# ZhiHuangHn/vtkCloudPoint

Measured on AMD Instinct MI355X. Metric: Mpoints/s DBSCAN+label @10M pts, higher is better.
Workload: dtype f64; 1 GPU; C4: 10000000-pt cloud (half uniform background, 200 Gaussian blobs), one monolithic DBImproved.dbscan, metric L1_2D, eps 0.1, minPts 10; mode=single, points_total=10000000, points_per_gpu=10000000, clusters=27380, resident_in_hbm=True

## Files before the change

### vtkcloudpoint_amd/csrc/dbscan.hip

```cpp
#include <string.h>

#include <cmath>
#include <cstdlib>
#include <cstring>
#include <limits>
#include <vector>

#include "bounds.hpp"
#include "dbscan_engine.hpp"
#include "grid_common.hpp"

using namespace vcpg;

namespace {

#ifndef VCP_UNR2
#define VCP_UNR2 4
#endif
#ifndef VCP_UNR3
#define VCP_UNR3 2
#endif
#ifndef VCP_UNRW
#define VCP_UNRW 4
#endif
// ... 814 lines not shown
template <bool FILTER>
__global__ __launch_bounds__(TPB) void k_flatten(uint32_t* __restrict__ parent, const uint32_t* __restrict__ sord,
                                                uint32_t* __restrict__ minord, WorkList wlE) {
  const uint32_t p = wl_fetch(wlE);
  uint32_t r = NONE, v = NONE;
  if (p != NONE) {
    r = (uint32_t)p;
    uint32_t x = parent[r];
    while (x != r) {
      r = x;
      x = parent[r];
    }
    parent[p] = r;
    v = sord[p];
  }
  unsigned long long todo = __ballot(r != NONE);
  const int lane = threadIdx.x & 63;
  while (todo) {
    int leader = __ffsll((long long)todo) - 1;
    uint32_t lr = __shfl(r, leader, 64);
    bool mine = (r == lr);
    uint32_t m = mine ? v : NONE;
#pragma unroll
    for (int d = 32; d > 0; d >>= 1) m = min(m, (uint32_t)__shfl_xor((int)m, d, 64));
    if (lane == leader &&
        (!FILTER || m < __hip_atomic_load(&minord[lr], __ATOMIC_RELAXED, __HIP_MEMORY_SCOPE_AGENT)))
      atomicMin(&minord[lr], m);
    todo &= ~__ballot(mine);
  }
}

__device__ __forceinline__ uint32_t seed_rank(const uint32_t* __restrict__ bits, const uint32_t* __restrict__ pref,
                                              uint32_t m) {
  const uint32_t w = m >> 5;
  return pref[w] + (uint32_t)__popc(bits[w] & ((1u << (m & 31u)) - 1u));
}
__global__ __launch_bounds__(TPB) void k_seed_popc(const uint32_t* __restrict__ bits, uint32_t nw, uint32_t* __restrict__ cnt) {
  uint32_t w = blockIdx.x * TPB + threadIdx.x;
  if (w < nw) cnt[w] = (uint32_t)__popc(bits[w]);
}

__global__ __launch_bounds__(TPB) void k_seedflag(const uint32_t* __restrict__ parent, const uint32_t* __restrict__ minord,
                                                 uint32_t* __restrict__ seedflag, WorkList wlE) {
  const uint32_t p = wl_fetch(wlE);
  if (p == NONE) return;
  if (parent[p] == p) {
    const uint32_t m = minord[p];
    atomicOr(&seedflag[m >> 5], 1u << (m & 31u));
  }
}

__global__ __launch_bounds__(TPB) void k_rootk(const uint32_t* __restrict__ parent, const uint32_t* __restrict__ minord,
                                              const uint32_t* __restrict__ seedbits, const uint32_t* __restrict__ seedpref,
                                              uint32_t* __restrict__ rootk, uint32_t* __restrict__ clseed, WorkList wlE) {
  const uint32_t p = wl_fetch(wlE);
  if (p == NONE) return;
  if (parent[p] == p) {
    uint32_t k = seed_rank(seedbits, seedpref, minord[p]);
    rootk[p] = k;
    clseed[k] = minord[p];
  }
}

__device__ __forceinline__ void twice_add(unsigned twice, unsigned long long* __restrict__ counters) {
  __shared__ unsigned tw[TPB / 64];
  const unsigned long long m2 = __ballot(twice);
  if ((threadIdx.x & 63) == 0) tw[threadIdx.x >> 6] = (unsigned)__popcll(m2);
  __syncthreads();
  if (threadIdx.x == 0) {
    unsigned t = 0;
    for (int k = 0; k < TPB / 64; k++) t += tw[k];
    if (t) atomicAdd(&counters[36 + (blockIdx.x & 31)], (unsigned long long)t);
  }
}

template <int GD, int METRIC, bool GROUPED>
__global__ __launch_bounds__(TPB) void k_border(ExactSrc xs, GridP g, double thr,
                                               CellTab ct,
                                               const int32_t* __restrict__ sgroup, const uint8_t* __restrict__ flags,
                                               const uint32_t* __restrict__ parent, const uint32_t* __restrict__ sord,
                                               const uint32_t* __restrict__ rootk, const uint32_t* __restrict__ clseed,
                                               uint32_t* __restrict__ labk, unsigned long long* __restrict__ counters,
                                               uint32_t* __restrict__ group_twice, WorkList wlB, uint32_t own_lo,
                                               uint32_t own_span, const float* __restrict__ sorted32, Screen sc) {
  const uint32_t p = wl_fetch(wlB);
  unsigned twice = 0;
  if (p != NONE) {
    const uint8_t fl = flags[p];
    uint32_t out = 0;
    {
      float qf[3];
      int cc[3];
      load_pt32<GD>(sorted32, p, qf);
      cell_of32<GD>(qf, g, cc);
      constexpr int UNR = VCP_UNRW;
      const int32_t myg = GROUPED ? sgroup[p] : 0;
      uint32_t mx = 0, mnk = NONE;
      for_rows<GD>(cc, g, ct, [&](uint32_t s, uint32_t e) {
        for (uint32_t j0 = s; j0 < e; j0 += UNR) {
          uint32_t rk[UNR];
#pragma unroll
          for (int u = 0; u < UNR; u++) rk[u] = rootk[min(j0 + u, e - 1)];
#pragma unroll
          for (int u = 0; u < UNR; u++) {
            const uint32_t j = j0 + u, x = rk[u];
            if (j >= e || x == NONE || (x >= mnk && x < mx)) continue;
            if (GROUPED && sgroup[j] != myg) continue;
            float rr[3];
            load_pt32<GD>(sorted32, j, rr);
            if (within_scr<GD, METRIC>(qf, rr, sc, xs, p, j, thr)) {
              mx = max(mx, x + 1u);
              mnk = min(mnk, x);
            }
          }
        }
        return true;
      });
      out = mx;
      if (mx != 0 && !(fl & F_CLASSED) && sord[p] - own_lo < own_span && sord[p] < clseed[mnk]) {
        twice = 1;
        if (GROUPED) atomicAdd(&group_twice[myg], 1u);
      }
    }
    labk[p] = (out << 2) | ((fl & F_CORE) ? 1u : 0u) | ((fl & F_CLASSED) ? 2u : 0u);
  }
  if (!GROUPED) twice_add(twice, counters);
}

template <bool GROUPED>
__global__ __launch_bounds__(TPB) void k_border_list(const int32_t* __restrict__ sgroup, const uint8_t* __restrict__ flags,
                                                    const uint32_t* __restrict__ sord, const uint32_t* __restrict__ rootk,
                                                    const uint32_t* __restrict__ clseed, uint32_t* __restrict__ labk,
                                                    unsigned long long* __restrict__ counters,
                                                    uint32_t* __restrict__ group_twice, NbrOut no, WorkList wlB) {
  const uint32_t p = wl_fetch(wlB);
  unsigned twice = 0;
  if (p != NONE) {
    const uint8_t fl = flags[p];
    const int nrec = fl >> 4;
    uint32_t mx = 0, mnk = NONE;
    const uint32_t* li = nbr_list(no, p);
    for (int k = 0; k < nrec; k++) {
      const uint32_t x = rootk[li[k]];
      if (x == NONE) continue;
      mx = max(mx, x + 1u);
      mnk = min(mnk, x);
    }
    if (mx != 0 && sord[p] < clseed[mnk]) twice = 1;
    labk[p] = (mx << 2) | ((fl & F_CORE) ? 1u : 0u) | ((fl & F_CLASSED) ? 2u : 0u);
  }
  if (GROUPED) {
    const int32_t g = twice ? sgroup[p] : -1;
    unsigned long long todo = __ballot(twice != 0);
    const int lane = threadIdx.x & 63;
    while (todo) {
      const int leader = __ffsll((long long)todo) - 1;
      const int32_t gl = __shfl(g, leader, 64);
      const unsigned long long same = __ballot(twice && g == gl);
      if (lane == leader) atomicAdd(&group_twice[gl], (uint32_t)__popcll(same));
      todo &= ~same;
    }
  } else {
    twice_add(twice, counters);
  }
}

__global__ __launch_bounds__(TPB) void k_labk_rest(const uint8_t* __restrict__ flags, const uint32_t* __restrict__ parent,
                                                  uint32_t* rootk, uint32_t* __restrict__ labk,
                                                  CellTab ct) {
  const uint32_t nin = *ct.nin;
  int64_t p = (int64_t)blockIdx.x * TPB + threadIdx.x;
  if (p >= nin) return;
  const uint8_t fl = flags[p];
  uint32_t k = NONE;
  if (fl & F_EXPAND) {
    const uint32_t r = parent[p];
    k = rootk[r];
    if (r != (uint32_t)p) rootk[p] = k;
  } else {
    rootk[p] = NONE;
  }
  if (fl & F_BCAND) return;
  const uint32_t out = (fl & F_EXPAND) ? k + 1u : 0u;
  labk[p] = (out << 2) | ((fl & F_CORE) ? 1u : 0u) | ((fl & F_CLASSED) ? 2u : 0u);
}

template <bool GROUPED>
__global__ __launch_bounds__(TPB) void k_output(int64_t n, const uint32_t* __restrict__ pos,
                                               const uint32_t* __restrict__ labk,
                                               const uint8_t* __restrict__ in_classed, const int32_t* __restrict__ group,
                                               const uint32_t* __restrict__ groupstart,
                                               const uint32_t* __restrict__ seedbits,
                                               const uint32_t* __restrict__ seedpref, int32_t cf_in,
                                               int32_t* __restrict__ labels, uint8_t* __restrict__ is_core,
                                               uint8_t* __restrict__ is_classed,
                                               unsigned long long* __restrict__ counters) {
  int64_t i = (int64_t)blockIdx.x * TPB + threadIdx.x;
  unsigned unclassed = 0;
  (void)counters;
  if (i < n) {
    const uint32_t p = pos[i];
    if (p == NONE) {
      if (GROUPED) return;
      if (!in_classed) labels[i] = 0;
      if (is_core) is_core[i] = 0;
      if (is_classed) is_classed[i] = in_classed ? in_classed[i] : 0;
    } else {
      const uint32_t w = labk[p];
      const uint32_t k1 = w >> 2;
      const bool core = w & 1u, classed = w & 2u;
      int32_t lab = 0;
      if (k1) {
        uint32_t base = GROUPED ? seed_rank(seedbits, seedpref, groupstart[group[i]]) : 0u;
        lab = cf_in + (int32_t)(k1 - base);
      }
      if (lab != 0 || !in_classed) labels[i] = lab;
      if (is_core) is_core[i] = (core && !classed) ? 1 : 0;
      if (is_classed) is_classed[i] = (classed || lab != 0) ? 1 : 0;
      if (!classed) unclassed = 1;
    }
  }
  if (in_classed) {
    __shared__ unsigned wcnt[TPB / 64];
    unsigned long long m1 = __ballot(unclassed);
    if ((threadIdx.x & 63) == 0) wcnt[threadIdx.x >> 6] = (unsigned)__popcll(m1);
    __syncthreads();
    if (threadIdx.x == 0) {
// ... 431 lines not shown
    static const int cap_env = getenv("VCP_CORE_CAP") ? atoi(getenv("VCP_CORE_CAP")) : -1;
    no.core_cap = (GD == 2 && (uint64_t)n < (uint64_t)g.ncells) ? std::min(no.NB, CORE_LIST) : no.NB;
    if (cap_env >= 0) no.core_cap = std::min(no.NB, cap_env);
  }
  const size_t lds_nb = (size_t)no.NB * TPB * 4;
  static const bool core_global = getenv("VCP_CORE_GLOBAL") != nullptr;
  if constexpr (GD == 2) {
    if (!GROUPED || !core_global)
      VCP_LAUNCH(ctx, (k_core_lds<GD, METRIC, GROUPED>), dim3(nb), dim3(TPB), 0, st, xs, g, thr, min_pts, ct, sgroup, flags,
                      parent, minord, blkE, blkB, no, sorted32, sc, flags_set);
    else
      VCP_LAUNCH(ctx, (k_core<GD, METRIC, GROUPED>), dim3(nb), dim3(TPB), 2 * lds_nb, st, xs, g, thr, min_pts, ct,
                      sgroup, flags, parent, minord, blkE, blkB, no, sorted32, sc, flags_set);
  } else
    VCP_LAUNCH(ctx, (k_core<GD, METRIC, GROUPED>), dim3(nb), dim3(TPB), 2 * lds_nb, st, xs, g, thr, min_pts, ct,
                    sgroup, flags, parent, minord, blkE, blkB, no, sorted32, sc, flags_set);
  VCP_TRY(vcp_exclusive_scan_u32(ctx, blkE, blkE, 2 * ((int64_t)nb + 2), nullptr));
  VCP_LAUNCH(ctx, k_wl_fill, dim3(nb), dim3(TPB), 0, st, flags, ct, blkE, blkB, wlE.list, wlB.list,
                  seedflag, nw, counters, GROUPED ? ext->d_group_twice : nullptr, (uint32_t)(GROUPED ? G : 0));

  vcp_phase(ctx, "union");
  const bool pre = GD == 2 || no.NB > 0;
  if (no.NB > 0) {
    VCP_LAUNCH(ctx, k_union_init_list, dim3(nbl), dim3(TPB), 0, st, flags, parent, no, wlE);
    static const int join_all = getenv("VCP_JOIN_ALL") ? atoi(getenv("VCP_JOIN_ALL")) : -1;
    const bool all = join_all >= 0 ? join_all != 0 : (uint64_t)n >= (uint64_t)g.ncells;
    if (all) VCP_LAUNCH(ctx, k_flatten0<2>, dim3(nbl), dim3(TPB), 0, st, parent, wlE, flags, no);
    else VCP_LAUNCH(ctx, k_flatten0<1>, dim3(nbl), dim3(TPB), 0, st, parent, wlE, flags, no);
    VCP_LAUNCH(ctx, k_flatten0<0>, dim3(nbl), dim3(TPB), 0, st, parent, wlE, flags, no);
  } else if (GD == 2) {
    VCP_LAUNCH(ctx, (k_union_init<GD, METRIC, GROUPED>), dim3(nbl), dim3(TPB), 0, st, xs, g, thr, ct, sgroup,
                    flags, parent, wlE, sorted32, sc);
    VCP_LAUNCH(ctx, k_flatten0<0>, dim3(nbl), dim3(TPB), 0, st, parent, wlE, flags, no);
  }
  const bool dense = pre && (uint64_t)n > (uint64_t)DENSE_PER_CELL * g.ncells;
  if (dense) {
    VCP_TRY(vcp_ensure(ctx, ctx->b_aux0, ((size_t)nb * (TPB / 64) + 2) * 4));
    uint32_t* chunkroot = ctx->b_aux0.as<uint32_t>();
    VCP_LAUNCH(ctx, k_chunkroot, dim3(nb), dim3(TPB), 0, st, parent, ct, chunkroot);
    VCP_LAUNCH(ctx, (k_union<GD, METRIC, GROUPED, true, true>), dim3(nbl), dim3(TPB), 0, st, xs, g, thr, ct, sgroup,
                    parent, wlE, sorted32, sc, chunkroot);
  } else if (pre)
    VCP_LAUNCH(ctx, (k_union<GD, METRIC, GROUPED, true>), dim3(nbl), dim3(TPB), 0, st, xs, g, thr, ct, sgroup,
                    parent, wlE, sorted32, sc);
  else
    VCP_LAUNCH(ctx, (k_union<GD, METRIC, GROUPED, false>), dim3(nbl), dim3(TPB), 0, st, xs, g, thr, ct, sgroup,
                    parent, wlE, sorted32, sc);
  vcp_phase(ctx, "flatten_number");
  if ((uint64_t)n >= (uint64_t)g.ncells)
    VCP_LAUNCH(ctx, k_flatten<true>, dim3(nbl), dim3(TPB), 0, st, parent, sord, minord, wlE);
  else
    VCP_LAUNCH(ctx, k_flatten<false>, dim3(nbl), dim3(TPB), 0, st, parent, sord, minord, wlE);
  if (!GROUPED && ext && ext->slab) {
    vcp_phase(ctx, "slab_components");
    VCP_LAUNCH(ctx, k_slab_count, dim3(nb), dim3(TPB), 0, st, parent, flags, ct, blkE);
    VCP_TRY(vcp_exclusive_scan_u32(ctx, blkE, blkE, (int64_t)nb + 1, nullptr));
    VCP_LAUNCH(ctx, k_slab_fill, dim3(nb), dim3(TPB), 0, st, parent, flags, minord, ct, blkE, clseed);
    VCP_LAUNCH(ctx, k_slab_out, dim3(nb), dim3(TPB), 0, st, n, pos, flags, parent, minord, ext->d_slab_rep, d_is_core);
    uint32_t* hn = reinterpret_cast<uint32_t*>(ctx->pinned) + 64;
    VCP_HIP(ctx, hipMemcpyAsync(hn, blkE + nb, 4, hipMemcpyDeviceToHost, st));
    VCP_TRY(vcp_phase_finish(ctx));
    VCP_HIP(ctx, hipStreamSynchronize(st));
    if (!ctx->slab) ctx->slab = new SlabState();
    SlabState& ss = *ctx->slab;
    ss.valid = true;
    ss.gd = GD;
    ss.metric = METRIC;
    ss.n = n;
    ss.n_comp = hn[0];
    ss.g = g;
    ss.thr = thr;
    ss.sc = sc;
    ss.xs = xs;
    ss.nb = nb;
    if (cf_out) *cf_out = (int32_t)hn[0];
    return VCP_OK;
  }
  VCP_LAUNCH(ctx, k_seedflag, dim3(nbl), dim3(TPB), 0, st, parent, minord, seedflag, wlE);
  VCP_LAUNCH(ctx, k_seed_popc, dim3(vcp_blocks(nw, TPB)), dim3(TPB), 0, st, seedflag, nw, seedpref);
  VCP_TRY(vcp_exclusive_scan_u32(ctx, seedpref, seedpref, nw, d_total));
  VCP_LAUNCH(ctx, k_rootk, dim3(nbl), dim3(TPB), 0, st, parent, minord, seedflag, seedpref, rootk, clseed, wlE);

  vcp_phase(ctx, "border");
  VCP_LAUNCH(ctx, k_labk_rest, dim3(nb), dim3(TPB), 0, st, flags, parent, rootk, labk, ct);
  if (no.NB > 0)
    VCP_LAUNCH(ctx, k_border_list<GROUPED>, dim3(nbl), dim3(TPB), 0, st, sgroup, flags, sord, rootk, clseed, labk, counters,
                    GROUPED ? ext->d_group_twice : nullptr, no, wlB);
  else
    VCP_LAUNCH(ctx, (k_border<GD, METRIC, GROUPED>), dim3(nbl), dim3(TPB), 0, st, xs, g, thr, ct, sgroup, flags,
                    parent, sord, rootk, clseed, labk, counters, GROUPED ? ext->d_group_twice : nullptr, wlB, 0u, NONE,
                    sorted32, sc);
  if (part_out) {
    GridOutputArgs oa;
    oa.n = n;
    oa.sord = sord;
    oa.labk = labk;
    oa.have_in_classed = d_in_classed != nullptr;
    oa.cf_in = cf_in;
    oa.labels = d_labels;
    oa.is_core = d_is_core;
    oa.is_classed = d_is_classed;
    oa.counters = counters;
    VCP_TRY(vcp_grid_output_partition(ctx, oa));
  } else {
    vcp_phase(ctx, "output");
    VCP_LAUNCH(ctx, (k_output<GROUPED>), dim3(nb), dim3(TPB), 0, st, n, pos, labk, d_in_classed, d_group,
                    GROUPED ? ext->d_groupstart : nullptr, seedflag, seedpref, cf_in, d_labels, d_is_core, d_is_classed,
                    counters);
  }
  if (!GROUPED && min_pts <= 0 && !all_finite)
    VCP_LAUNCH(ctx, k_lonely_seeds<GD>, dim3(nb), dim3(TPB), 0, st, d_coords, n, stride, d_in_classed, d_is_classed,
                    counters);
  if (GROUPED) {
    VCP_LAUNCH(ctx, k_group_stats, dim3(vcp_blocks(G, TPB)), dim3(TPB), 0, st, G, glo, ghi, ext->d_groupstart,
                    seedflag, seedpref, ext->d_group_twice, ext->d_group_nclus, counters + 3, ext->skip_upto);
    if (ext->d_group_evals)
      VCP_HIP(ctx, hipMemcpyAsync(ext->d_group_evals, counters + 3, 8, hipMemcpyDeviceToDevice, st));
  }
  unsigned long long* hc = reinterpret_cast<unsigned long long*>(ctx->pinned) + 8;
  VCP_HIP(ctx, hipMemcpyAsync(hc, counters, 68 * sizeof(unsigned long long), hipMemcpyDeviceToHost, st));
  VCP_TRY(vcp_phase_finish(ctx));
  VCP_HIP(ctx, hipStreamSynchronize(st));
  const uint32_t K = *reinterpret_cast<uint32_t*>(hc + 2);
  unsigned long long unclassed = (unsigned long long)n;
  if (d_in_classed) {
    unclassed = 0;
    for (int k = 0; k < 32; k++) unclassed += hc[4 + k];
  }
  if (cf_out) *cf_out = cf_in + (int32_t)K;
  unsigned long long twice_total = 0;
  for (int k = 0; k < 32; k++) twice_total += hc[36 + k];
  if (dist_evals) *dist_evals = GROUPED ? (int64_t)hc[3] : (int64_t)(unclassed + twice_total + K - hc[0]) * n;
  return VCP_OK;
}

template <int GD, int METRIC>
int run_slab_finish(vcp_ctx* ctx, const SlabState& ss, const uint32_t* d_map_rep, const uint32_t* d_map_k,
                    const int32_t* d_tab_gid, uint32_t own_lo, uint32_t own_span, int32_t* d_labels,
                    uint8_t* d_is_classed, int64_t* twice) {
  hipStream_t st = ctx->stream;
  const int64_t n = ss.n;
  const unsigned nb = ss.nb;
  const GridP g = ss.g;
  const size_t ctw = vcp_ct_words(g.ncells);
  const CellTab ct{ctx->b_ctw.as<uint4>(), ctx->b_ctd.as<uint32_t>(),
                   reinterpret_cast<uint32_t*>(ctx->b_ctw.as<char>() + ctw * 16) + 1};
  uint32_t* pos = ctx->b_pos.as<uint32_t>();
  uint32_t* sord = ctx->b_sidx.as<uint32_t>();
  uint8_t* flags = ctx->b_flags.as<uint8_t>();
  uint32_t* parent = ctx->b_parent.as<uint32_t>();
  uint32_t* minord = ctx->b_minord.as<uint32_t>();
  uint32_t* rootk = ctx->b_rootcl.as<uint32_t>();
  uint32_t* clseed = ctx->b_clseed.as<uint32_t>();
  uint32_t* labk = ctx->b_labk.as<uint32_t>();
  WorkList wlB;
  uint32_t* blkE = ctx->b_wl.as<uint32_t>();
  uint32_t* blkB = blkE + (nb + 2);
  wlB.list = blkB + (nb + 2) + n;
  wlB.scan = blkB;
  wlB.nblk = nb;
  wlB.perblk = list_perblk(n);
  const unsigned nbl = 8u * LCHUNK * wlB.perblk;
  const int rb = (int)vcp_blocks(n, TPB, 1024);
  unsigned long long* counters = reinterpret_cast<unsigned long long*>(ctx->b_misc.as<double>() + (size_t)rb * 8 + 8);
  vcp_phase(ctx, "slab_roots");
  VCP_HIP(ctx, hipMemsetAsync(counters, 0, 68 * sizeof(unsigned long long), st));
  VCP_LAUNCH(ctx, k_slab_rootk, dim3(nb), dim3(TPB), 0, st, parent, flags, minord, ct, d_map_rep, d_map_k,
                  (uint32_t)ss.n_comp, rootk, counters);
  vcp_phase(ctx, "border");
  VCP_LAUNCH(ctx, k_labk_rest, dim3(nb), dim3(TPB), 0, st, flags, parent, rootk, labk, ct);
  VCP_LAUNCH(ctx, (k_border<GD, METRIC, false>), dim3(nbl), dim3(TPB), 0, st, ss.xs, g, ss.thr,
                  ct, nullptr, flags, parent, sord, rootk, clseed, labk, counters, nullptr, wlB, own_lo, own_span,
                  ctx->b_sorted32.as<float>(), ss.sc);
  vcp_phase(ctx, "output");
  VCP_LAUNCH(ctx, k_slab_output, dim3(nb), dim3(TPB), 0, st, n, pos, labk, d_tab_gid, d_labels, d_is_classed);
  unsigned long long* hc = reinterpret_cast<unsigned long long*>(ctx->pinned) + 8;
  VCP_HIP(ctx, hipMemcpyAsync(hc, counters, 68 * sizeof(unsigned long long), hipMemcpyDeviceToHost, st));
  VCP_TRY(vcp_phase_finish(ctx));
  VCP_HIP(ctx, hipStreamSynchronize(st));
  if (hc[0] != 0)
    return vcp_fail(ctx, VCP_ERR_ARG, "%llu local components are missing from the map", hc[0]);
  if (twice) {
    *twice = 0;
    for (int k = 0; k < 32; k++) *twice += (int64_t)hc[36 + k];
  }
  return VCP_OK;
}

int run_degenerate(vcp_ctx* ctx, int64_t n, int min_pts, int32_t cf_in, const uint8_t* d_in_classed,
                   int32_t* d_labels, uint8_t* d_is_core, uint8_t* d_is_classed, int32_t* cf_out,
                   int64_t* dist_evals) {
  hipStream_t st = ctx->stream;
  const unsigned nb = vcp_blocks(n, TPB);
  vcp_phase(ctx, "degenerate");
  VCP_TRY(vcp_ensure(ctx, ctx->b_seedflag, (size_t)(n + 2) * 4));
  VCP_TRY(vcp_ensure(ctx, ctx->b_misc, 64));
  uint32_t* f = ctx->b_seedflag.as<uint32_t>();
  uint32_t* d_total = ctx->b_misc.as<uint32_t>();
  VCP_LAUNCH(ctx, k_unclassed_flag, dim3(nb), dim3(TPB), 0, st, d_in_classed, f, n);
  VCP_TRY(vcp_exclusive_scan_u32(ctx, f, f, n, d_total));
  const int all_core = 0 >= min_pts;
  VCP_LAUNCH(ctx, k_degenerate, dim3(nb), dim3(TPB), 0, st, d_in_classed, f, n, cf_in, all_core,
                  d_in_classed == nullptr, d_labels, d_is_core, d_is_classed);
  uint32_t* hu = reinterpret_cast<uint32_t*>(ctx->pinned);
  VCP_HIP(ctx, hipMemcpyAsync(hu, d_total, 4, hipMemcpyDeviceToHost, st));
  VCP_TRY(vcp_phase_finish(ctx));
  VCP_HIP(ctx, hipStreamSynchronize(st));
  if (cf_out) *cf_out = cf_in + (all_core ? (int32_t)hu[0] : 0);
  if (dist_evals) *dist_evals = (int64_t)hu[0] * n;
  return VCP_OK;
}

}

int vcp_dbscan_engine(vcp_ctx* ctx, const double* d_coords, int64_t n, int stride, int metric, double eps,
                      int min_pts, int32_t cf_in, const uint8_t* d_in_classed, int32_t* d_labels,
                      uint8_t* d_is_core, uint8_t* d_is_classed, int32_t* cf_out, int64_t* dist_evals,
                      const DbscanExt* ext) {
  if (!ctx) return VCP_ERR_ARG;
  if (n < 0) return vcp_fail(ctx, VCP_ERR_ARG, "n < 0");
  if (stride != 2 && stride != 3) return vcp_fail(ctx, VCP_ERR_ARG, "dim must be 2 or 3");
  if (metric < 0 || metric > 3) return vcp_fail(ctx, VCP_ERR_ARG, "unknown metric %d", metric);
  if (metric == VCP_SIGNED_SUM_2D) {
    if (ext) return vcp_fail(ctx, VCP_ERR_ARG, "DB has no grouped / staged form");
    if (n >= 0x7FFFFFF0LL) return vcp_fail(ctx, VCP_ERR_TOO_LARGE, "n beyond 32-bit indexing");
    if (n > 0 && (!d_coords || !d_labels)) return vcp_fail(ctx, VCP_ERR_ARG, "null buffer");
    VCP_TRY(vcp_bind(ctx));
    vcp_phase_reset(ctx);
    if (ctx->slab) ctx->slab->valid = false;
    if (n == 0) {
      if (cf_out) *cf_out = cf_in;
      if (dist_evals) *dist_evals = 0;
      ctx->last_timing.clear();
      return VCP_OK;
    }
    return vcp_db_engine(ctx, d_coords, n, stride, eps, min_pts, cf_in, nullptr, d_in_classed, d_labels, d_is_core,
                         d_is_classed, cf_out, dist_evals);
  }
  if (metric == VCP_L2_3D && stride != 3) return vcp_fail(ctx, VCP_ERR_ARG, "VCP_L2_3D needs dim 3");
  if (n >= 0x3FFFFFF0LL) return vcp_fail(ctx, VCP_ERR_TOO_LARGE, "n beyond 30-bit indexing");
  if (n > 0 && (!d_coords || !d_labels)) return vcp_fail(ctx, VCP_ERR_ARG, "null buffer");
  const bool grouped = ext && ext->d_group;
  if (grouped && (metric != VCP_L1_2D || !ext->d_groupstart || !ext->d_group_twice || d_in_classed))
    return vcp_fail(ctx, VCP_ERR_ARG, "grouped DBSCAN needs groupstart, group_twice and the L1 metric");
  VCP_TRY(vcp_bind(ctx));
  vcp_phase_reset(ctx);
  if (ctx->slab) ctx->slab->valid = false;
  if (n == 0) {
    if (cf_out) *cf_out = cf_in;
    if (dist_evals) *dist_evals = 0;
    ctx->last_timing.clear();
    return VCP_OK;
  }
  if (!(eps >= 0.0)) {
    if (grouped) return vcp_fail(ctx, VCP_ERR_ARG, "grouped DBSCAN needs eps >= 0");
    return run_degenerate(ctx, n, min_pts, cf_in, d_in_classed, d_labels, d_is_core, d_is_classed, cf_out, dist_evals);
// ... 154 lines not shown
```

### vtkcloudpoint_amd/csrc/grid_common.hpp

```cpp
#pragma once
#include "vcp_ctx.hpp"

namespace vcpg {

constexpr int TPB = 256;
constexpr uint8_t F_CORE = 1, F_CLASSED = 2, F_EXPAND = 4, F_BCAND = 8;
constexpr uint32_t NONE = 0xFFFFFFFFu;

struct GridP {
  double mn[3];
  double inv_h;
  double scale;
  int D[3];
  uint32_t ncells;
};

template <int GD>
__device__ __forceinline__ uint32_t cell_id(const GridP& g, int cx, int cy, int cz) {
  uint32_t id = (uint32_t)cy * (uint32_t)g.D[0] + (uint32_t)cx;
  if (GD == 3) id += (uint32_t)cz * (uint32_t)g.D[0] * (uint32_t)g.D[1];
  return id;
}

__device__ __forceinline__ float rel32(double x, double mn, double scale) { return (float)((x - mn) * scale); }
// ... 76 lines not shown
  return t.dense[(size_t)w.w * 32u + i];
}
__device__ __forceinline__ uint32_t ct_from_word(const CellTab& t, const uint4 w, uint32_t cell) {
  const uint32_t i = cell & 31u, below = (1u << i) - 1u;
  if ((w.x & w.y & below) == 0u) return w.z + (uint32_t)__popc(w.x & below) + 2u * (uint32_t)__popc(w.y & below);
  return t.dense[(size_t)w.w * 32u + i];
}
__device__ __forceinline__ void ct_range(const CellTab& t, uint32_t c0, uint32_t c1, uint32_t& s, uint32_t& e) {
  const uint4 w0 = t.words[c0 >> 5];
  s = ct_from_word(t, w0, c0);
  e = (c1 >> 5) == (c0 >> 5) ? ct_from_word(t, w0, c1) : ct_start(t, c1);
}

struct Screen {
  float lo, hi;
};

template <int GD>
__device__ __forceinline__ void load_pt32(const float* __restrict__ c, int64_t i, float* q) {
  if (GD == 2) {
    const float2 v = *reinterpret_cast<const float2*>(c + 2 * i);
    q[0] = v.x;
    q[1] = v.y;
  } else {
    const float4 v = *reinterpret_cast<const float4*>(c + 4 * i);
    q[0] = v.x;
    q[1] = v.y;
    q[2] = v.z;
  }
}
template <int GD>
__device__ __forceinline__ void store_pt32(float* __restrict__ c, int64_t i, const double* q, const GridP& g) {
  if (GD == 2) {
    *reinterpret_cast<float2*>(c + 2 * i) = make_float2(rel32(q[0], g.mn[0], g.scale), rel32(q[1], g.mn[1], g.scale));
  } else {
    *reinterpret_cast<float4*>(c + 4 * i) =
        make_float4(rel32(q[0], g.mn[0], g.scale), rel32(q[1], g.mn[1], g.scale), rel32(q[2], g.mn[2], g.scale), 0.0f);
  }
}

struct ExactSrc {
  const double* base;
  const uint32_t* idx;
  int stride;
};
template <int GD>
__device__ __forceinline__ void load_exact(const ExactSrc& xs, uint32_t p, double* q) {
  const int64_t i = xs.idx ? (int64_t)xs.idx[p] : (int64_t)p;
  load_in<GD>(xs.base, i, xs.stride, q);
}

}

struct GridBuildArgs {
  const double* d_coords = nullptr;
  int64_t n = 0;
  int stride = 2, gd = 2;
  vcpg::GridP g;
  const int32_t* d_group = nullptr;
  int glo = 0, ghi = 0;
  const uint32_t* d_ord = nullptr;
  const uint8_t* d_in_classed = nullptr;
  uint4* ctwords = nullptr;
  uint32_t* ctdense = nullptr;
  uint32_t* ctcount = nullptr;
  float* sorted32 = nullptr;
  uint32_t* sord = nullptr;
  uint32_t* sidx = nullptr;
  int32_t* sgroup = nullptr;
  uint8_t* flags = nullptr;
  uint32_t* pos = nullptr;
};
__host__ __device__ static inline size_t vcp_ct_words(uint32_t ncells) { return ((size_t)ncells + 32) / 32; }
static inline size_t vcp_ct_dense_cap(int64_t n, uint32_t ncells) {
  const size_t w = vcp_ct_words(ncells), byn = (size_t)n / 3 + 1;
  return w < byn ? w : byn;
}
int vcp_grid_build_partition(vcp_ctx* ctx, const GridBuildArgs& a);

struct GridOutputArgs {
  int64_t n = 0;
  const uint32_t* sord = nullptr;
  const uint32_t* labk = nullptr;
  bool have_in_classed = false;
  int32_t cf_in = 0;
  int32_t* labels = nullptr;
  uint8_t* is_core = nullptr;
  uint8_t* is_classed = nullptr;
  unsigned long long* counters = nullptr;
};
int vcp_grid_output_partition(vcp_ctx* ctx, const GridOutputArgs& a);
```

### vtkcloudpoint_amd/csrc/gridbuild.hip

```cpp
#include <algorithm>
#include <mutex>
#include <unordered_map>

#include "grid_common.hpp"

using namespace vcpg;

namespace {

constexpr int PT = 1024;
constexpr int PCH_MIN = 8192;
constexpr int FT = 1024;
constexpr uint32_t MAXB = 8192;
constexpr uint32_t wcap(int) { return 4096u; }
constexpr uint32_t QUEUE_FROM = 32;

typedef float4 Rec;

template <int GD>
__device__ __forceinline__ Rec rec_make(const float* qf, uint32_t idx, uint32_t cell) {
  return GD == 2 ? make_float4(qf[0], qf[1], __uint_as_float(idx), __uint_as_float(cell))
                 : make_float4(qf[0], qf[1], qf[2], __uint_as_float(idx));
}
template <int GD>
// ... 494 lines not shown
      uint32_t i;
      const uint32_t p = cnt[padded(rec_cell<GD>(r, g, i) - c0)] + rk[j] - s - w0;
      if (p < WCAP) stage_put<GD>(s32, sidx, p, r, i);
    }
    __syncthreads();
    fine_flush<GD, GROUPED>(s + w0, min(WCAP, m - w0), s32, sidx, ord, in_classed, group, sorted32, sord, sidx_out, sgroup,
                            flags, pos);
    __syncthreads();
  }
}

template <int GD, bool GROUPED>
__global__ __launch_bounds__(FT) void k_part_fine_windows(const Rec* __restrict__ rec, const uint32_t* __restrict__ rk,
                                                         const uint32_t* __restrict__ bstart, uint32_t bstride,
                                                         const uint32_t* __restrict__ total, uint32_t B, GridP g,
                                                         const uint32_t* __restrict__ ord, const uint8_t* __restrict__ in_classed,
                                                         const int32_t* __restrict__ group, CellTab ct,
                                                         float* __restrict__ sorted32,
                                                         uint32_t* __restrict__ sord, uint32_t* __restrict__ sidx_out,
                                                         int32_t* __restrict__ sgroup, uint8_t* __restrict__ flags,
                                                         uint32_t* __restrict__ pos, const uint2* __restrict__ queue,
                                                         const uint32_t* __restrict__ qcount) {
  extern __shared__ __attribute__((aligned(16))) unsigned char lds[];
  constexpr uint32_t WCAP = wcap(GD);
  constexpr uint32_t FPR = GD == 2 ? 2 : 4;
  float* s32 = reinterpret_cast<float*>(lds);
  uint32_t* sidx = reinterpret_cast<uint32_t*>(s32 + (size_t)WCAP * FPR);
  const uint32_t nq = *qcount;
  for (uint32_t qi = blockIdx.x; qi < nq; qi += gridDim.x) {
    const uint2 q = queue[qi];
    const uint32_t b = q.x, w0 = q.y;
    uint32_t s, e;
    bucket_range(bstart, bstride, total, b, B, s, e);
    const uint32_t m = e - s;
    for (uint32_t j = s + threadIdx.x; j < e; j += FT) {
      const Rec r = rec[j];
      uint32_t i;
      const uint32_t p = ct_start(ct, rec_cell<GD>(r, g, i)) + rk[j] - s - w0;
      if (p < WCAP) stage_put<GD>(s32, sidx, p, r, i);
    }
    __syncthreads();
    fine_flush<GD, GROUPED>(s + w0, min(WCAP, m - w0), s32, sidx, ord, in_classed, group, sorted32, sord, sidx_out, sgroup,
                            flags, pos);
    __syncthreads();
  }
}

constexpr int OT = 1024, OPT = 16;
constexpr int OWT = 512;

template <int OWSH>
__global__ __launch_bounds__(OT) void k_out_scatter(const uint32_t* __restrict__ sord, const uint32_t* __restrict__ labk,
                                                   int64_t n, uint32_t OB, uint32_t* __restrict__ gcur,
                                                   uint2* __restrict__ rec) {
  extern __shared__ uint32_t h[];
  for (uint32_t k = threadIdx.x; k < OB; k += OT) h[k] = 0;
  __syncthreads();
  const int64_t first = (int64_t)blockIdx.x * (OT * OPT);
  uint32_t o[OPT], w[OPT], r[OPT];
#pragma unroll
  for (int k = 0; k < OPT; k++) {
    const int64_t p = first + (int64_t)k * OT + threadIdx.x;
    o[k] = NONE;
    if (p < n) {
      o[k] = sord[p];
      w[k] = labk[p];
      r[k] = atomicAdd(&h[o[k] >> OWSH], 1u);
    }
  }
  __syncthreads();
  for (uint32_t k = threadIdx.x; k < OB; k += OT) {
    const uint32_t c = h[k];
    if (c) h[k] = atomicAdd(&gcur[k], c);
  }
  __syncthreads();
#pragma unroll
  for (int k = 0; k < OPT; k++) {
    if (o[k] == NONE) continue;
    const uint32_t bk = o[k] >> OWSH;
    rec[((size_t)bk << OWSH) + h[bk] + r[k]] = make_uint2(o[k], w[k]);
  }
}

template <int OWSH>
__global__ __launch_bounds__(OWT) void k_out_write(const uint2* __restrict__ rec, int64_t n, bool have_in_classed,
                                                  int32_t cf_in, int32_t* __restrict__ labels,
                                                  uint8_t* __restrict__ is_core, uint8_t* __restrict__ is_classed,
                                                  unsigned long long* __restrict__ counters, uint32_t* __restrict__ gcur) {
  extern __shared__ __attribute__((aligned(16))) uint32_t sw[];
  if (threadIdx.x == 0) gcur[blockIdx.x] = 0u;
  const int64_t lo = (int64_t)blockIdx.x << OWSH;
  const uint32_t cnt = (uint32_t)min((int64_t)1 << OWSH, n - lo);
  unsigned unclassed = 0;
  for (uint32_t j = threadIdx.x; j < cnt; j += OWT) {
    const uint2 v = rec[lo + j];
    sw[v.x - (uint32_t)lo] = v.y;
    if (!(v.y & 2u)) unclassed++;
  }
  __syncthreads();
  auto lab_of = [&](uint32_t w) { return (w >> 2) ? cf_in + (int32_t)(w >> 2) : 0; };
  auto core_of = [](uint32_t w) { return (uint32_t)((w & 3u) == 1u); };
  auto cls_of = [](uint32_t w) { return (uint32_t)((w & 2u) != 0u || (w >> 2) != 0u); };
  const bool vec = (((uintptr_t)labels & 15u) | ((uintptr_t)is_core & 3u) | ((uintptr_t)is_classed & 3u)) == 0;
  const uint32_t c4 = vec ? cnt >> 2 : 0u;
  for (uint32_t j = threadIdx.x; j < c4; j += OWT) {
    const uint4 w = reinterpret_cast<const uint4*>(sw)[j];
    const int4 l = make_int4(lab_of(w.x), lab_of(w.y), lab_of(w.z), lab_of(w.w));
    if (have_in_classed) {
      if (l.x) labels[lo + 4 * j] = l.x;
      if (l.y) labels[lo + 4 * j + 1] = l.y;
      if (l.z) labels[lo + 4 * j + 2] = l.z;
      if (l.w) labels[lo + 4 * j + 3] = l.w;
    } else {
      reinterpret_cast<int4*>(labels + lo)[j] = l;
    }
    if (is_core)
      reinterpret_cast<uint32_t*>(is_core + lo)[j] = core_of(w.x) | core_of(w.y) << 8 | core_of(w.z) << 16 | core_of(w.w) << 24;
    if (is_classed)
      reinterpret_cast<uint32_t*>(is_classed + lo)[j] = cls_of(w.x) | cls_of(w.y) << 8 | cls_of(w.z) << 16 | cls_of(w.w) << 24;
  }
  for (uint32_t j = (c4 << 2) + threadIdx.x; j < cnt; j += OWT) {
    const uint32_t w = sw[j];
    const int32_t l = lab_of(w);
    if (!have_in_classed || l) labels[lo + j] = l;
    if (is_core) is_core[lo + j] = (uint8_t)core_of(w);
    if (is_classed) is_classed[lo + j] = (uint8_t)cls_of(w);
  }
  if (have_in_classed) {
    __shared__ unsigned wc[OWT / 64];
#pragma unroll
    for (int d = 32; d > 0; d >>= 1) unclassed += __shfl_down(unclassed, d, 64);
    if ((threadIdx.x & 63) == 0) wc[threadIdx.x >> 6] = unclassed;
    __syncthreads();
    if (threadIdx.x == 0) {
      unsigned t = 0;
      for (int k = 0; k < OWT / 64; k++) t += wc[k];
      if (t) atomicAdd(&counters[4 + (blockIdx.x & 31)], (unsigned long long)t);
    }
  }
}

int allow_lds(vcp_ctx* ctx, const void* kernel, size_t bytes) {
  static std::mutex mu;
  static std::unordered_map<uint64_t, size_t> allowed;
  std::lock_guard<std::mutex> lk(mu);
  const uint64_t key = (uint64_t)reinterpret_cast<uintptr_t>(kernel) * 64u + (uint64_t)(ctx->device & 63);
  size_t& have = allowed.emplace(key, (size_t)64 * 1024).first->second;
  if (bytes > have) {
    VCP_HIP(ctx, hipFuncSetAttribute(kernel, hipFuncAttributeMaxDynamicSharedMemorySize, (int)bytes));
    have = bytes;
  }
  return VCP_OK;
}
template <class K>
int allow_lds(vcp_ctx* ctx, K kernel, size_t bytes) {
  return allow_lds(ctx, reinterpret_cast<const void*>(kernel), bytes);
}

template <int GD, bool GROUPED>
int build(vcp_ctx* ctx, const GridBuildArgs& a) {
  hipStream_t st = ctx->stream;
  const PartGeom pg = part_geom(a.n, a.g.ncells);
  const size_t nc = (size_t)pg.NS * pg.nchunk;
  VCP_TRY(vcp_ensure(ctx, ctx->b_hist, (nc + 8) * 4));
  VCP_TRY(vcp_ensure(ctx, ctx->b_rec, (size_t)a.n * sizeof(Rec)));
  uint32_t* counts = ctx->b_hist.as<uint32_t>();
  uint32_t* total = counts + nc;
  Rec* rec = ctx->b_rec.as<Rec>();
  const size_t lds_h = (size_t)pg.NS * 4;
  const uint32_t CPB = 1u << pg.csh;
  const size_t lds_f = ((((size_t)CPB + CPB / 32) + 4) & ~3ull) * 4 + (size_t)wcap(GD) * ((GD == 2 ? 8 : 16) + 4);
  VCP_TRY(allow_lds(ctx, k_part_fine<GD, GROUPED>, lds_f));
  VCP_TRY(vcp_ensure(ctx, ctx->b_fineq, ((size_t)a.n / wcap(GD) + pg.B + 8) * sizeof(uint2) + 64));
  uint32_t* qcount = ctx->b_fineq.as<uint32_t>();
  uint2* queue = reinterpret_cast<uint2*>(ctx->b_fineq.as<char>() + 64);
  vcp_phase(ctx, "part_hist");
  const uint32_t csh_a = pg.csh + pg.a;
  VCP_LAUNCH(ctx, (k_part_hist<GD, GROUPED>), dim3(pg.nchunk), dim3(PT), lds_h, st, a.d_coords, a.n, a.stride, a.g,
                  a.d_group, a.glo, a.ghi, csh_a, pg.NS, pg.chunk, pg.nchunk, counts, qcount, a.ctcount);
  VCP_TRY(vcp_exclusive_scan_u32(ctx, counts, counts, (int64_t)nc, total));
  vcp_phase(ctx, "part_scatter");
  VCP_LAUNCH(ctx, (k_part_scatter<GD, GROUPED>), dim3(pg.nchunk), dim3(PT), lds_h, st, a.d_coords, a.n, a.stride, a.g,
                  a.d_group, a.glo, a.ghi, csh_a, pg.NS, pg.chunk, pg.nchunk, counts, rec, a.pos);
  const uint32_t* bstart = counts;
  uint32_t bstride = pg.nchunk;
  if (pg.a > 0) {
    vcp_phase(ctx, "part_split");
    VCP_TRY(vcp_ensure(ctx, ctx->b_rec2, (size_t)a.n * sizeof(Rec)));
    VCP_TRY(vcp_ensure(ctx, ctx->b_bstart, ((size_t)pg.B + 2) * 4));
    VCP_LAUNCH(ctx, k_part_split<GD>, dim3(pg.NS), dim3(FT), 0, st, rec, ctx->b_rec2.as<Rec>(), counts, total, pg.nchunk,
                    pg.NS, pg.a, pg.csh, pg.B, a.g, ctx->b_bstart.as<uint32_t>());
    rec = ctx->b_rec2.as<Rec>();
    bstart = ctx->b_bstart.as<uint32_t>();
    bstride = 1;
  }
  vcp_phase(ctx, "part_fine");
  VCP_TRY(vcp_ensure(ctx, ctx->b_rank, (size_t)a.n * 4));
  VCP_TRY(vcp_ensure(ctx, ctx->b_bstate, (size_t)pg.B + 16));
  uint8_t* bstate = ctx->b_bstate.as<uint8_t>();
  VCP_LAUNCH(ctx, (k_part_fine_small<GD, GROUPED>), dim3(pg.B), dim3(FS), 0, st, rec, bstart, bstride, total, pg.B, pg.csh,
                  a.g, a.d_ord, a.d_in_classed, a.d_group, a.ctwords, a.ctdense, a.ctcount, bstate, a.sorted32, a.sord,
                  a.sidx, a.sgroup, a.flags, a.pos);
  VCP_LAUNCH(ctx, (k_part_fine<GD, GROUPED>), dim3(pg.B), dim3(FT), lds_f, st, rec, ctx->b_rank.as<uint32_t>(), bstart,
                  bstride, total, pg.B, pg.csh, a.g, a.d_ord, a.d_in_classed, a.d_group, a.ctwords, a.ctdense, a.ctcount,
                  a.sorted32, a.sord, a.sidx, a.sgroup, a.flags, a.pos, queue, qcount, bstate);
  {
    const size_t lds_w = (size_t)wcap(GD) * ((GD == 2 ? 8 : 16) + 4);
    VCP_TRY(allow_lds(ctx, k_part_fine_windows<GD, GROUPED>, lds_w));
    const unsigned gw = (unsigned)std::min<size_t>(768, (size_t)a.n / wcap(GD) + 1);
    const CellTab ct{a.ctwords, a.ctdense, a.ctcount + 1};
    VCP_LAUNCH(ctx, (k_part_fine_windows<GD, GROUPED>), dim3(gw), dim3(FT), lds_w, st, rec, ctx->b_rank.as<uint32_t>(),
                    bstart, bstride, total, pg.B, a.g, a.d_ord, a.d_in_classed, a.d_group, ct, a.sorted32,
                    a.sord, a.sidx, a.sgroup, a.flags, a.pos, queue, qcount);
  }
  return VCP_OK;
}

}

int vcp_grid_build_partition(vcp_ctx* ctx, const GridBuildArgs& a) {
  const bool grouped = a.d_group != nullptr;
  if (a.gd == 3) {
    if (grouped) return vcp_fail(ctx, VCP_ERR_ARG, "grouped calls are 2-D");
    return build<3, false>(ctx, a);
  }
  return grouped ? build<2, true>(ctx, a) : build<2, false>(ctx, a);
}

template <int OWSH>
static int output_partition(vcp_ctx* ctx, const GridOutputArgs& a) {
  hipStream_t st = ctx->stream;
  const uint32_t OB = (uint32_t)((a.n + (1 << OWSH) - 1) >> OWSH);
  const void* before = ctx->b_outcur.p;
  const size_t before_cap = ctx->b_outcur.cap;
  VCP_TRY(vcp_ensure(ctx, ctx->b_outcur, ((size_t)OB + 8) * 4));
  if (ctx->b_outcur.p != before || ctx->b_outcur.cap != before_cap)
    VCP_HIP(ctx, hipMemsetAsync(ctx->b_outcur.p, 0, ctx->b_outcur.cap, st));
  VCP_TRY(vcp_ensure(ctx, ctx->b_rec, (size_t)OB << (OWSH + 3)));
  uint32_t* gcur = ctx->b_outcur.as<uint32_t>();
  uint2* rec = ctx->b_rec.as<uint2>();
  VCP_TRY(allow_lds(ctx, k_out_write<OWSH>, (size_t)4 << OWSH));
  vcp_phase(ctx, "out_scatter");
  VCP_LAUNCH(ctx, k_out_scatter<OWSH>, dim3(vcp_blocks(a.n, OT * OPT)), dim3(OT), (size_t)OB * 4, st, a.sord, a.labk, a.n,
                  OB, gcur, rec);
  vcp_phase(ctx, "out_write");
  VCP_LAUNCH(ctx, k_out_write<OWSH>, dim3(OB), dim3(OWT), (size_t)4 << OWSH, st, rec, a.n, a.have_in_classed, a.cf_in,
                  a.labels, a.is_core, a.is_classed, a.counters, gcur);
  return VCP_OK;
}

int vcp_grid_output_partition(vcp_ctx* ctx, const GridOutputArgs& a) {
  if (a.n > ((int64_t)1 << 27)) return vcp_fail(ctx, VCP_ERR_TOO_LARGE, "more than 2^27 points: use the gather output");
  if (a.n >= ((int64_t)1 << 23)) return output_partition<15>(ctx, a);
  if (a.n >= ((int64_t)1 << 22)) return output_partition<14>(ctx, a);
  return output_partition<13>(ctx, a);
}
```

Baseline: 6996 Mpoints/s.

## Skip labk fill pass and scatter only labeled points in partitioned output

When the partitioned output path is used without an input isClassed array, the separate k_labk_rest pass is dropped. Border kernels now resolve cluster ids through parent->rootk. A new sparse scatter kernel emits records only for border candidates and expanded points, computing their label word on the fly, and the write kernel zero-fills its shared tile and reads only the emitted record count. This cuts a full pass over all points and shrinks the record traffic for noise points, at the cost of an extra indirect load per neighbour and an extra LDS clear.

Result: faster. 7274 Mpoints/s (median of 6 runs) (+4.0%).

```diff
diff --git a/vtkcloudpoint_amd/csrc/dbscan.hip b/vtkcloudpoint_amd/csrc/dbscan.hip
--- a/vtkcloudpoint_amd/csrc/dbscan.hip
+++ b/vtkcloudpoint_amd/csrc/dbscan.hip
@@ -920,7 +920,8 @@
                                                const uint32_t* __restrict__ rootk, const uint32_t* __restrict__ clseed,
                                                uint32_t* __restrict__ labk, unsigned long long* __restrict__ counters,
                                                uint32_t* __restrict__ group_twice, WorkList wlB, uint32_t own_lo,
-                                               uint32_t own_span, const float* __restrict__ sorted32, Screen sc) {
+                                               uint32_t own_span, const float* __restrict__ sorted32, Screen sc,
+                                               bool via_parent) {
   const uint32_t p = wl_fetch(wlB);
   unsigned twice = 0;
   if (p != NONE) {
@@ -938,7 +939,12 @@
         for (uint32_t j0 = s; j0 < e; j0 += UNR) {
           uint32_t rk[UNR];
 #pragma unroll
-          for (int u = 0; u < UNR; u++) rk[u] = rootk[min(j0 + u, e - 1)];
+          for (int u = 0; u < UNR; u++) rk[u] = via_parent ? parent[min(j0 + u, e - 1)] : rootk[min(j0 + u, e - 1)];
+          if (via_parent) {
+#pragma unroll
+            for (int u = 0; u < UNR; u++)
+              if (rk[u] != NONE) rk[u] = rootk[rk[u]];
+          }
 #pragma unroll
           for (int u = 0; u < UNR; u++) {
             const uint32_t j = j0 + u, x = rk[u];
@@ -965,8 +971,9 @@
   if (!GROUPED) twice_add(twice, counters);
 }
 
-template <bool GROUPED>
+template <bool GROUPED, bool VIA_PARENT>
 __global__ __launch_bounds__(TPB) void k_border_list(const int32_t* __restrict__ sgroup, const uint8_t* __restrict__ flags,
+                                                    const uint32_t* __restrict__ parent,
                                                     const uint32_t* __restrict__ sord, const uint32_t* __restrict__ rootk,
                                                     const uint32_t* __restrict__ clseed, uint32_t* __restrict__ labk,
                                                     unsigned long long* __restrict__ counters,
@@ -979,8 +986,9 @@
     uint32_t mx = 0, mnk = NONE;
     const uint32_t* li = nbr_list(no, p);
     for (int k = 0; k < nrec; k++) {
-      const uint32_t x = rootk[li[k]];
+      uint32_t x = VIA_PARENT ? parent[li[k]] : rootk[li[k]];
       if (x == NONE) continue;
+      if (VIA_PARENT) x = rootk[x];
       mx = max(mx, x + 1u);
       mnk = min(mnk, x);
     }
@@ -1578,19 +1586,28 @@
   VCP_LAUNCH(ctx, k_rootk, dim3(nbl), dim3(TPB), 0, st, parent, minord, seedflag, seedpref, rootk, clseed, wlE);
 
   vcp_phase(ctx, "border");
-  VCP_LAUNCH(ctx, k_labk_rest, dim3(nb), dim3(TPB), 0, st, flags, parent, rootk, labk, ct);
-  if (no.NB > 0)
-    VCP_LAUNCH(ctx, k_border_list<GROUPED>, dim3(nbl), dim3(TPB), 0, st, sgroup, flags, sord, rootk, clseed, labk, counters,
-                    GROUPED ? ext->d_group_twice : nullptr, no, wlB);
+  const bool sparse_out = part_out && !d_in_classed && getenv("VCP_OUT_ALL") == nullptr;
+  if (!sparse_out) VCP_LAUNCH(ctx, k_labk_rest, dim3(nb), dim3(TPB), 0, st, flags, parent, rootk, labk, ct);
+  if (no.NB > 0 && sparse_out)
+    VCP_LAUNCH(ctx, (k_border_list<GROUPED, true>), dim3(nbl), dim3(TPB), 0, st, sgroup, flags, parent, sord, rootk, clseed,
+                    labk, counters, GROUPED ? ext->d_group_twice : nullptr, no, wlB);
+  else if (no.NB > 0)
+    VCP_LAUNCH(ctx, (k_border_list<GROUPED, false>), dim3(nbl), dim3(TPB), 0, st, sgroup, flags, parent, sord, rootk, clseed,
+                    labk, counters, GROUPED ? ext->d_group_twice : nullptr, no, wlB);
   else
     VCP_LAUNCH(ctx, (k_border<GD, METRIC, GROUPED>), dim3(nbl), dim3(TPB), 0, st, xs, g, thr, ct, sgroup, flags,
                     parent, sord, rootk, clseed, labk, counters, GROUPED ? ext->d_group_twice : nullptr, wlB, 0u, NONE,
-                    sorted32, sc);
+                    sorted32, sc, sparse_out);
   if (part_out) {
     GridOutputArgs oa;
     oa.n = n;
     oa.sord = sord;
     oa.labk = labk;
+    if (sparse_out) {
+      oa.flags = flags;
+      oa.parent = parent;
+      oa.rootk = rootk;
+    }
     oa.have_in_classed = d_in_classed != nullptr;
     oa.cf_in = cf_in;
     oa.labels = d_labels;
@@ -1667,7 +1684,7 @@
   VCP_LAUNCH(ctx, k_labk_rest, dim3(nb), dim3(TPB), 0, st, flags, parent, rootk, labk, ct);
   VCP_LAUNCH(ctx, (k_border<GD, METRIC, false>), dim3(nbl), dim3(TPB), 0, st, ss.xs, g, ss.thr,
                   ct, nullptr, flags, parent, sord, rootk, clseed, labk, counters, nullptr, wlB, own_lo, own_span,
-                  ctx->b_sorted32.as<float>(), ss.sc);
+                  ctx->b_sorted32.as<float>(), ss.sc, false);
   vcp_phase(ctx, "output");
   VCP_LAUNCH(ctx, k_slab_output, dim3(nb), dim3(TPB), 0, st, n, pos, labk, d_tab_gid, d_labels, d_is_classed);
   unsigned long long* hc = reinterpret_cast<unsigned long long*>(ctx->pinned) + 8;
diff --git a/vtkcloudpoint_amd/csrc/grid_common.hpp b/vtkcloudpoint_amd/csrc/grid_common.hpp
--- a/vtkcloudpoint_amd/csrc/grid_common.hpp
+++ b/vtkcloudpoint_amd/csrc/grid_common.hpp
@@ -182,6 +182,9 @@
   int64_t n = 0;
   const uint32_t* sord = nullptr;
   const uint32_t* labk = nullptr;
+  const uint8_t* flags = nullptr;
+  const uint32_t* parent = nullptr;
+  const uint32_t* rootk = nullptr;
   bool have_in_classed = false;
   int32_t cf_in = 0;
   int32_t* labels = nullptr;
diff --git a/vtkcloudpoint_amd/csrc/gridbuild.hip b/vtkcloudpoint_amd/csrc/gridbuild.hip
--- a/vtkcloudpoint_amd/csrc/gridbuild.hip
+++ b/vtkcloudpoint_amd/csrc/gridbuild.hip
@@ -600,17 +600,75 @@
   }
 }
 
+constexpr int SOPT = 8;
 template <int OWSH>
+__global__ __launch_bounds__(OT) void k_out_scatter_sparse(const uint32_t* __restrict__ sord, const uint32_t* __restrict__ labk,
+                                                          const uint8_t* __restrict__ flags,
+                                                          const uint32_t* __restrict__ parent,
+                                                          const uint32_t* __restrict__ rootk, int64_t n, uint32_t OB,
+                                                          uint32_t* __restrict__ gcur, uint2* __restrict__ rec) {
+  extern __shared__ uint32_t h[];
+  for (uint32_t k = threadIdx.x; k < OB; k += OT) h[k] = 0;
+  __syncthreads();
+  const uint32_t base = blockIdx.x * (uint32_t)(OT * SOPT) + threadIdx.x, nn = (uint32_t)n;
+  uint32_t o[SOPT], w[SOPT], r[SOPT], fl[SOPT];
+#pragma unroll
+  for (int k = 0; k < SOPT; k++) {
+    const uint32_t p = base + (uint32_t)k * OT;
+    fl[k] = flags[min(p, nn - 1u)];
+    if (p >= nn) fl[k] = 0u;
+  }
+#pragma unroll
+  for (int k = 0; k < SOPT; k++) {
+    const uint32_t p = base + (uint32_t)k * OT;
+    w[k] = 0;
+    o[k] = NONE;
+    if (fl[k] & F_BCAND) w[k] = labk[p];
+    if ((fl[k] & (F_BCAND | F_EXPAND)) == F_EXPAND) w[k] = parent[p];
+    if (fl[k] & (F_BCAND | F_EXPAND)) o[k] = sord[p];
+  }
+#pragma unroll
+  for (int k = 0; k < SOPT; k++)
+    if ((fl[k] & (F_BCAND | F_EXPAND)) == F_EXPAND) w[k] = ((rootk[w[k]] + 1u) << 2) | ((fl[k] & F_CORE) ? 1u : 0u);
+#pragma unroll
+  for (int k = 0; k < SOPT; k++) {
+    r[k] = 0;
+    if (w[k] == 0) o[k] = NONE;
+    if (w[k] != 0) r[k] = atomicAdd(&h[o[k] >> OWSH], 1u);
+  }
+  __syncthreads();
+  for (uint32_t k = threadIdx.x; k < OB; k += OT) {
+    const uint32_t c = h[k];
+    if (c) h[k] = atomicAdd(&gcur[k], c);
+  }
+  __syncthreads();
+#pragma unroll
+  for (int k = 0; k < SOPT; k++) {
+    if (o[k] == NONE) continue;
+    const uint32_t bk = o[k] >> OWSH;
+    rec[((size_t)bk << OWSH) + h[bk] + r[k]] = make_uint2(o[k], w[k]);
+  }
+}
+
+template <int OWSH, bool SPARSE>
 __global__ __launch_bounds__(OWT) void k_out_write(const uint2* __restrict__ rec, int64_t n, bool have_in_classed,
                                                   int32_t cf_in, int32_t* __restrict__ labels,
                                                   uint8_t* __restrict__ is_core, uint8_t* __restrict__ is_classed,
                                                   unsigned long long* __restrict__ counters, uint32_t* __restrict__ gcur) {
   extern __shared__ __attribute__((aligned(16))) uint32_t sw[];
-  if (threadIdx.x == 0) gcur[blockIdx.x] = 0u;
   const int64_t lo = (int64_t)blockIdx.x << OWSH;
   const uint32_t cnt = (uint32_t)min((int64_t)1 << OWSH, n - lo);
+  uint32_t nrec = cnt;
+  if (SPARSE) {
+    __shared__ uint32_t scnt;
+    if (threadIdx.x == 0) scnt = gcur[blockIdx.x];
+    for (uint32_t j = threadIdx.x; j < (cnt + 3u) >> 2; j += OWT) reinterpret_cast<uint4*>(sw)[j] = make_uint4(0u, 0u, 0u, 0u);
+    __syncthreads();
+    nrec = min(scnt, cnt);
+  }
+  if (threadIdx.x == 0) gcur[blockIdx.x] = 0u;
   unsigned unclassed = 0;
-  for (uint32_t j = threadIdx.x; j < cnt; j += OWT) {
+  for (uint32_t j = threadIdx.x; j < nrec; j += OWT) {
     const uint2 v = rec[lo + j];
     sw[v.x - (uint32_t)lo] = v.y;
     if (!(v.y & 2u)) unclassed++;
@@ -757,13 +815,24 @@
   VCP_TRY(vcp_ensure(ctx, ctx->b_rec, (size_t)OB << (OWSH + 3)));
   uint32_t* gcur = ctx->b_outcur.as<uint32_t>();
   uint2* rec = ctx->b_rec.as<uint2>();
-  VCP_TRY(allow_lds(ctx, k_out_write<OWSH>, (size_t)4 << OWSH));
+  const bool sparse = a.flags != nullptr;
+  if (sparse && a.have_in_classed) return vcp_fail(ctx, VCP_ERR_ARG, "the sparse output takes no isClassed input");
+  if (sparse) VCP_TRY(allow_lds(ctx, k_out_write<OWSH, true>, (size_t)4 << OWSH));
+  else VCP_TRY(allow_lds(ctx, k_out_write<OWSH, false>, (size_t)4 << OWSH));
   vcp_phase(ctx, "out_scatter");
-  VCP_LAUNCH(ctx, k_out_scatter<OWSH>, dim3(vcp_blocks(a.n, OT * OPT)), dim3(OT), (size_t)OB * 4, st, a.sord, a.labk, a.n,
-                  OB, gcur, rec);
+  if (sparse)
+    VCP_LAUNCH(ctx, k_out_scatter_sparse<OWSH>, dim3(vcp_blocks(a.n, OT * SOPT)), dim3(OT), (size_t)OB * 4, st, a.sord, a.labk,
+                    a.flags, a.parent, a.rootk, a.n, OB, gcur, rec);
+  else
+    VCP_LAUNCH(ctx, k_out_scatter<OWSH>, dim3(vcp_blocks(a.n, OT * OPT)), dim3(OT), (size_t)OB * 4, st, a.sord, a.labk, a.n,
+                    OB, gcur, rec);
   vcp_phase(ctx, "out_write");
-  VCP_LAUNCH(ctx, k_out_write<OWSH>, dim3(OB), dim3(OWT), (size_t)4 << OWSH, st, rec, a.n, a.have_in_classed, a.cf_in,
-                  a.labels, a.is_core, a.is_classed, a.counters, gcur);
+  if (sparse)
+    VCP_LAUNCH(ctx, (k_out_write<OWSH, true>), dim3(OB), dim3(OWT), (size_t)4 << OWSH, st, rec, a.n, false, a.cf_in,
+                    a.labels, a.is_core, a.is_classed, a.counters, gcur);
+  else
+    VCP_LAUNCH(ctx, (k_out_write<OWSH, false>), dim3(OB), dim3(OWT), (size_t)4 << OWSH, st, rec, a.n, a.have_in_classed,
+                    a.cf_in, a.labels, a.is_core, a.is_classed, a.counters, gcur);
   return VCP_OK;
 }
 
```
